# snap-stanford/KGWAS

Measured on AMD Instinct MI355X. Metric: edges aggregated/sec (full fast-mode KG minibatch training; epoch time in config), higher is better.
Workload: dtype f32

## Files before the change

kgwas_amd/csrc/kgw_dense_linear.h:

```cpp
#pragma once

namespace {

constexpr int LBM = 128, LBN = 128, LBK = 32, LPAD = 33;

struct LinArgs {
    const float* X; int64_t ldx;
    const float* W; int64_t ldw;
    const float* bias;
    const float* mask;
    int64_t ldm;
    float* Y; int64_t ldy;
    int64_t rows; int K, N;
    int relu, w_kn;
    const int32_t* rows_dev;
};

__device__ __forceinline__ int64_t lin_rows_eff(const LinArgs& a) {
    if (!a.rows_dev) return a.rows;
    const int64_t r = *a.rows_dev;
    return r < 0 ? 0 : (r < a.rows ? r : a.rows);
}

__device__ __forceinline__ void lin_zero_padding(const LinArgs& a, int64_t rows_eff, int64_t tid, int64_t nthreads) {
// ... 919 lines not shown
            const int idx = tid + 256 * it;
            const int k = idx & 127, n4 = (idx >> 7) * 4;
            Wl[(n4 + 0) * WST + k] = wv[it].x; Wl[(n4 + 1) * WST + k] = wv[it].y;
            Wl[(n4 + 2) * WST + k] = wv[it].z; Wl[(n4 + 3) * WST + k] = wv[it].w;
        }
    }
    __syncthreads();
    f32x4 bw[2][16];
#pragma unroll
    for (int t = 0; t < 2; ++t)
#pragma unroll
        for (int q = 0; q < 16; ++q) bw[t][q] = *(const f32x4*)(Wl + (t * 32 + li) * WST + lk * 64 + 4 * q);
    const float* w2 = Wl + (64 + li) * WST + lk * 64;
    const float* w3 = Wl + (96 + li) * WST + lk * 64;
    f32x16 accw[4];
#pragma unroll
    for (int t = 0; t < 4; ++t)
#pragma unroll
        for (int e = 0; e < 16; ++e) accw[t][e] = 0.f;
    const int K1 = a.K1;
    int tile = (int)blockIdx.x * 4 + wave;
    f32x4 xa[16];
    int src_cur;
    {
        int64_t r = (int64_t)(tile < ntiles ? tile : ntiles - 1) * 32 + li;
        if (r >= rows) r = rows - 1;
        src_cur = a.in_ids ? a.in_ids[r] : 0;
        const float* xp = a.dH2 + (a.in_ids ? (int64_t)(src_cur < 0 ? 0 : src_cur) : r) * a.ldd + lk * 64;
#pragma unroll
        for (int q = 0; q < 16; ++q) xa[q] = *(const f32x4*)(xp + 4 * q);
    }
    for (; tile < ntiles; tile += nw) {
        const int64_t r0 = (int64_t)tile * 32;
        const int64_t row = r0 + li;
        const bool live = row < rows && src_cur >= 0;
        const int64_t rc = row < rows ? row : rows - 1;
        const float* xn;
        {
            int nt = tile + nw;
            if (nt >= ntiles) nt = ntiles - 1;
            int64_t r = (int64_t)nt * 32 + li;
            if (r >= rows) r = rows - 1;
            src_cur = a.in_ids ? a.in_ids[r] : 0;
            xn = a.dH2 + (a.in_ids ? (int64_t)(src_cur < 0 ? 0 : src_cur) : r) * a.ldd + lk * 64;
        }
        float xs[16];
#pragma unroll
        for (int s2 = 0; s2 < 16; ++s2) {
            const int64_t rr = r0 + 2 * s2 + lk;
            float v = 0.f;
            if (rr < rows) v = li < K1 ? a.X[rr * a.ldx + li] : (li == K1 ? 1.f : 0.f);
            xs[s2] = v;
        }
        const float* mp = a.H1 + rc * a.ldm + 4 * lk;
        unsigned mb[2] = {0u, 0u};
        f32x4 mv[4];
#define KGW_MLPB_MFETCH(T)                                                                                \
        _Pragma("unroll") for (int g = 0; g < 4; ++g) mv[g] = *(const f32x4*)(mp + (T) * 32 + 8 * g);
#define KGW_MLPB_MBITS(T)                                                                                 \
        _Pragma("unroll") for (int g = 0; g < 4; ++g) {                                                  \
            const int b0 = ((T) & 1) * 16 + 4 * g;                                                        \
            mb[(T) >> 1] |= (mv[g].x > 0.f ? 1u : 0u) << (b0 + 0);                                        \
            mb[(T) >> 1] |= (mv[g].y > 0.f ? 1u : 0u) << (b0 + 1);                                        \
            mb[(T) >> 1] |= (mv[g].z > 0.f ? 1u : 0u) << (b0 + 2);                                        \
            mb[(T) >> 1] |= (mv[g].w > 0.f ? 1u : 0u) << (b0 + 3);                                        \
        }
        f32x16 acc[4];
#pragma unroll
        for (int t = 0; t < 4; ++t)
#pragma unroll
            for (int e = 0; e < 16; ++e) acc[t][e] = 0.f;
        f32x4 b2n = *(const f32x4*)w2, b3n = *(const f32x4*)w3;
#pragma unroll
        for (int q = 0; q < 16; ++q) {
            if (q == 0) { KGW_MLPB_MFETCH(0) }
            if (q == 3) { KGW_MLPB_MBITS(0) KGW_MLPB_MFETCH(1) }
            if (q == 6) { KGW_MLPB_MBITS(1) KGW_MLPB_MFETCH(2) }
            if (q == 10) { KGW_MLPB_MBITS(2) KGW_MLPB_MFETCH(3) }
            if (q == 14) { KGW_MLPB_MBITS(3) }
            const f32x4 b2 = b2n, b3 = b3n;
            if (q + 1 < 16) { b2n = *(const f32x4*)(w2 + 4 * (q + 1)); b3n = *(const f32x4*)(w3 + 4 * (q + 1)); }
#define KGW_MLPB_STEP(C)                                                                                  \
            acc[0] = __builtin_amdgcn_mfma_f32_32x32x2f32(bw[0][q].C, xa[q].C, acc[0], 0, 0, 0);          \
            acc[1] = __builtin_amdgcn_mfma_f32_32x32x2f32(bw[1][q].C, xa[q].C, acc[1], 0, 0, 0);          \
            acc[2] = __builtin_amdgcn_mfma_f32_32x32x2f32(b2.C, xa[q].C, acc[2], 0, 0, 0);                \
            acc[3] = __builtin_amdgcn_mfma_f32_32x32x2f32(b3.C, xa[q].C, acc[3], 0, 0, 0);
            KGW_MLPB_STEP(x) KGW_MLPB_STEP(y) KGW_MLPB_STEP(z) KGW_MLPB_STEP(w)
#undef KGW_MLPB_STEP
            if (q == 7) {
                __builtin_amdgcn_sched_barrier(0);
#pragma unroll
                for (int qq = 0; qq < 8; ++qq) xa[qq] = *(const f32x4*)(xn + 4 * qq);
                __builtin_amdgcn_sched_barrier(0);
            }
        }
#undef KGW_MLPB_MFETCH
#undef KGW_MLPB_MBITS
        if (!live) { mb[0] = 0u; mb[1] = 0u; }
        __builtin_amdgcn_sched_barrier(0);
#pragma unroll
        for (int qq = 8; qq < 16; ++qq) xa[qq] = *(const f32x4*)(xn + 4 * qq);
        __builtin_amdgcn_sched_barrier(0);
#pragma unroll
        for (int t = 0; t < 4; ++t)
#pragma unroll
            for (int g = 0; g < 4; ++g) {
                const unsigned m4 = mb[t >> 1] >> (((t & 1) << 4) + 4 * g);
                f32x4 v;
                v.x = (m4 & 1u) ? acc[t][4 * g + 0] : 0.f; v.y = (m4 & 2u) ? acc[t][4 * g + 1] : 0.f;
                v.z = (m4 & 4u) ? acc[t][4 * g + 2] : 0.f; v.w = (m4 & 8u) ? acc[t][4 * g + 3] : 0.f;
                *(f32x4*)(Tw + li * TST + t * 32 + 8 * g + 4 * lk) = v;
                if (a.dZ && row < rows) *(f32x4*)(a.dZ + row * a.ldz + t * 32 + 8 * g + 4 * lk) = v;
            }
        __asm__ volatile("s_waitcnt lgkmcnt(0)" ::: "memory");
#pragma unroll
        for (int s2 = 0; s2 < 16; ++s2) {
            const float* tp = Tw + (2 * s2 + lk) * TST + li;
#pragma unroll
            for (int t = 0; t < 4; ++t)
                accw[t] = __builtin_amdgcn_mfma_f32_32x32x2f32(xs[s2], tp[t * 32], accw[t], 0, 0, 0);
        }
        __asm__ volatile("s_waitcnt lgkmcnt(0)" ::: "memory");
    }
    __syncthreads();
    float* R = Tl;
#pragma unroll
    for (int t = 0; t < 4; ++t)
#pragma unroll
        for (int e = 0; e < 16; ++e) R[wave * 4096 + (t * 16 + e) * 64 + lane] = accw[t][e];
    __syncthreads();
    for (int f = tid; f < 4096; f += 256)
        a.part[(int64_t)blockIdx.x * 4096 + f] = (R[f] + R[4096 + f]) + (R[2 * 4096 + f] + R[3 * 4096 + f]);
}

constexpr int TS2 = 68;

template <bool PACK>
__global__ void __launch_bounds__(256) __attribute__((amdgpu_waves_per_eu(1, 1))) k_mlp2_bwd_first3(Mlp2BwdArgs a) {
    extern __shared__ __attribute__((aligned(16))) float lds[];
    uint4* W2p = (uint4*)lds;
    float* Tl = lds + M3_W2_U4 * 4;
    const int tid = threadIdx.x, lane = tid & 63, wave = tid >> 6;
    const int li = lane & 31, lk = lane >> 5;
    const unsigned sgn = (li & 1) ? 0x80000000u : 0u;
    int64_t rows = a.rows;
    if (a.rows_dev) { const int64_t r = *a.rows_dev; rows = r < 0 ? 0 : (r < a.rows ? r : a.rows); }
    if (rows == 0) {
        for (int f = tid; f < 4096; f += 256) a.part[(int64_t)blockIdx.x * 4096 + f] = 0.f;
        return;
    }
    const int ntiles = (int)((rows + 31) / 32);
    const int nw = (int)gridDim.x * 4;
    float* Tw = Tl + wave * 32 * TS2;
    for (int idx = tid; idx < 8 * 4 * 64; idx += 256) {
        const int ln = idx & 63, jt = (idx >> 6) & 3, s_ = idx >> 8;
        const float* wp = a.W2 + (int64_t)(64 * (ln >> 5) + 8 * s_) * a.ldw + 32 * jt + (ln & 31);
        float x[8];
#pragma unroll
        for (int i = 0; i < 8; ++i) x[i] = wp[(int64_t)i * a.ldw];
        uint4 p1, p2, p3;
        kgw_split3x8(x, p1, p2, p3);
        uint4* o = W2p + ((s_ * 3) * 4 + jt) * 64 + ln;
        o[0] = p1; o[4 * 64] = p2; o[8 * 64] = p3;
    }
    __syncthreads();
    const uint4* w2p = W2p + lane;
    f32x16 accw[4];
#pragma unroll
    for (int t = 0; t < 4; ++t)
#pragma unroll
        for (int e = 0; e < 16; ++e) accw[t][e] = 0.f;
    const int K1 = a.K1;
    int tile = (int)blockIdx.x * 4 + wave;
    f32x4 xa[16];
    int src_cur;
    {
        int64_t r = (int64_t)(tile < ntiles ? tile : ntiles - 1) * 32 + li;
        if (r >= rows) r = rows - 1;
        src_cur = a.in_ids ? a.in_ids[r] : 0;
        const float* xp = a.dH2 + (a.in_ids ? (int64_t)(src_cur < 0 ? 0 : src_cur) : r) * a.ldd + lk * 64;
#pragma unroll
        for (int q = 0; q < 16; ++q) xa[q] = *(const f32x4*)(xp + 4 * q);
    }
#define KGW_MLPB_BITS(MV, MB)                                                                            \
    _Pragma("unroll") for (int t_ = 0; t_ < 4; ++t_) _Pragma("unroll") for (int g = 0; g < 4; ++g) {    \
        const int b0 = (t_ & 1) * 16 + 4 * g;                                                            \
        MB[t_ >> 1] |= (MV[t_][g].x > 0.f ? 1u : 0u) << (b0 + 0);                                        \
        MB[t_ >> 1] |= (MV[t_][g].y > 0.f ? 1u : 0u) << (b0 + 1);                                        \
        MB[t_ >> 1] |= (MV[t_][g].z > 0.f ? 1u : 0u) << (b0 + 2);                                        \
        MB[t_ >> 1] |= (MV[t_][g].w > 0.f ? 1u : 0u) << (b0 + 3);                                        \
    }
    unsigned mb[2] = {0u, 0u};
    {
        int64_t r = (int64_t)(tile < ntiles ? tile : ntiles - 1) * 32 + li;
        if (r >= rows) r = rows - 1;
        const float* mp = a.H1 + r * a.ldm + 4 * lk;
        f32x4 mv[4][4];
#pragma unroll
        for (int t_ = 0; t_ < 4; ++t_)
#pragma unroll
            for (int g = 0; g < 4; ++g) mv[t_][g] = *(const f32x4*)(mp + t_ * 32 + 8 * g);
        KGW_MLPB_BITS(mv, mb)
    }
    for (; tile < ntiles; tile += nw) {
        const int64_t r0 = (int64_t)tile * 32;
        const int64_t row = r0 + li;
        const bool live = row < rows && src_cur >= 0;
        const int64_t rc = row < rows ? row : rows - 1;
        const float* xn;
        {
            int nt = tile + nw;
            if (nt >= ntiles) nt = ntiles - 1;
            int64_t r = (int64_t)nt * 32 + li;
            if (r >= rows) r = rows - 1;
            src_cur = a.in_ids ? a.in_ids[r] : 0;
            xn = a.dH2 + (a.in_ids ? (int64_t)(src_cur < 0 ? 0 : src_cur) : r) * a.ldd + lk * 64;
        }
        float xs[16];
#pragma unroll
        for (int s2 = 0; s2 < 16; ++s2) {
            const int64_t rr = r0 + 2 * s2 + lk;
            float v = 0.f;
            if (rr < rows) v = li < K1 ? a.X[rr * a.ldx + li] : (li == K1 ? 1.f : 0.f);
            xs[s2] = v;
        }
        f32x4 mvn[4][4];
        {
            int nt = tile + nw;
            if (nt >= ntiles) nt = ntiles - 1;
            int64_t r = (int64_t)nt * 32 + li;
            if (r >= rows) r = rows - 1;
            const float* mpn = a.H1 + r * a.ldm + 4 * lk;
#pragma unroll
            for (int t_ = 0; t_ < 4; ++t_)
#pragma unroll
                for (int g = 0; g < 4; ++g) mvn[t_][g] = *(const f32x4*)(mpn + t_ * 32 + 8 * g);
        }
        f32x16 acc[4];
#pragma unroll
        for (int t = 0; t < 4; ++t)
#pragma unroll
            for (int e = 0; e < 16; ++e) acc[t][e] = 0.f;
#pragma unroll
        for (int s_ = 0; s_ < 8; ++s_) {
            const f32x4 u = xa[2 * s_], v = xa[2 * s_ + 1];
            const float h[8] = {kgw_fxor(u.x, sgn), kgw_fxor(u.y, sgn), kgw_fxor(u.z, sgn), kgw_fxor(u.w, sgn),
                                kgw_fxor(v.x, sgn), kgw_fxor(v.y, sgn), kgw_fxor(v.z, sgn), kgw_fxor(v.w, sgn)};
            uint4 p1, p2, p3;
            kgw_split3x8(h, p1, p2, p3);
            const kgw_bf8 hb[3] = {__builtin_bit_cast(kgw_bf8, p1), __builtin_bit_cast(kgw_bf8, p2), __builtin_bit_cast(kgw_bf8, p3)};
            kgw_bf8 wa[3][4];
#pragma unroll
            for (int p = 0; p < 3; ++p)
#pragma unroll
                for (int jt = 0; jt < 4; ++jt) wa[p][jt] = __builtin_bit_cast(kgw_bf8, w2p[((s_ * 3 + p) * 4 + jt) * 64]);
            constexpr int TW[6] = {0, 2, 1, 0, 1, 0}, TH[6] = {2, 0, 1, 1, 0, 0};
#pragma unroll
            for (int t6 = 0; t6 < 6; ++t6)
#pragma unroll
                for (int jt = 0; jt < 4; ++jt)
                    acc[jt] = __builtin_amdgcn_mfma_f32_32x32x16_bf16(wa[TW[t6]][jt], hb[TH[t6]], acc[jt], 0, 0, 0);
            if (s_ == 3) {
                __builtin_amdgcn_sched_barrier(0);
#pragma unroll
                for (int qq = 0; qq < 8; ++qq) xa[qq] = *(const f32x4*)(xn + 4 * qq);
                __builtin_amdgcn_sched_barrier(0);
            }
        }
        if (!live) { mb[0] = 0u; mb[1] = 0u; }
        __builtin_amdgcn_sched_barrier(0);
#pragma unroll
        for (int qq = 8; qq < 16; ++qq) xa[qq] = *(const f32x4*)(xn + 4 * qq);
        __builtin_amdgcn_sched_barrier(0);
#pragma unroll
        for (int hh = 0; hh < 2; ++hh) {
#pragma unroll
            for (int t = 2 * hh; t < 2 * hh + 2; ++t)
#pragma unroll
                for (int g = 0; g < 4; ++g) {
                    const unsigned m4 = mb[t >> 1] >> (((t & 1) << 4) + 4 * g);
                    f32x4 v;
                    v.x = (m4 & 1u) ? kgw_fxor(acc[t][4 * g + 0], sgn) : 0.f; v.y = (m4 & 2u) ? kgw_fxor(acc[t][4 * g + 1], sgn) : 0.f;
                    v.z = (m4 & 4u) ? kgw_fxor(acc[t][4 * g + 2], sgn) : 0.f; v.w = (m4 & 8u) ? kgw_fxor(acc[t][4 * g + 3], sgn) : 0.f;
                    *(f32x4*)(Tw + li * TS2 + (t - 2 * hh) * 32 + 8 * g + 4 * lk) = v;
                    if (a.dZ && row < rows) *(f32x4*)(a.dZ + row * a.ldz + t * 32 + 8 * g + 4 * lk) = v;
                }
            __asm__ volatile("s_waitcnt lgkmcnt(0)" ::: "memory");
            if (PACK) {
                const bool neg = a.flip && ((tile / a.flip) & 1);
#pragma unroll
                for (int it = 0; it < 4; ++it) {
                    const int ntl = it & 1, j = it >> 1;
                    const float* tp = Tw + (16 * j + 8 * lk) * TS2 + 32 * ntl + li;
                    float x[8];
#pragma unroll
                    for (int i = 0; i < 8; ++i) x[i] = neg ? -tp[i * TS2] : tp[i * TS2];
                    uint4 p1, p2, p3;
                    kgw_split3x8(x, p1, p2, p3);
                    uint4* o = a.packed + (((int64_t)tile * 2 + j) * 3 * 4 + (2 * hh + ntl)) * 64 + lane;
                    o[0] = p1; o[4 * 64] = p2; o[8 * 64] = p3;
                }
            }
#pragma unroll
            for (int s2 = 0; s2 < 16; ++s2) {
                const float* tp = Tw + (2 * s2 + lk) * TS2 + li;
#pragma unroll
                for (int t = 0; t < 2; ++t)
                    accw[2 * hh + t] = __builtin_amdgcn_mfma_f32_32x32x2f32(xs[s2], tp[t * 32], accw[2 * hh + t], 0, 0, 0);
            }
            __asm__ volatile("s_waitcnt lgkmcnt(0)" ::: "memory");
        }
        mb[0] = 0u; mb[1] = 0u;
        KGW_MLPB_BITS(mvn, mb)
    }
#undef KGW_MLPB_BITS
    __syncthreads();
    float* R = lds;
#pragma unroll
    for (int t = 0; t < 4; ++t)
#pragma unroll
        for (int e = 0; e < 16; ++e) R[wave * 4096 + (t * 16 + e) * 64 + lane] = accw[t][e];
    __syncthreads();
    for (int f = tid; f < 4096; f += 256)
        a.part[(int64_t)blockIdx.x * 4096 + f] = (R[f] + R[4096 + f]) + (R[2 * 4096 + f] + R[3 * 4096 + f]);
}

__global__ void __launch_bounds__(1024) k_mlp2_bwd_fold(const float* __restrict__ part, int nblk, int K1, float* __restrict__ dW1,
                                                        int64_t ldw, float* __restrict__ db1) {
    __shared__ float sm[1024];
    const int fl = threadIdx.x & 63, g = threadIdx.x >> 6;
    const int f = blockIdx.x * 64 + fl;
    float s4[4] = {0.f, 0.f, 0.f, 0.f};
    int q = 0;
    for (int b = g; b < nblk; b += 16, ++q) s4[q & 3] += part[(int64_t)b * 4096 + f];
    sm[threadIdx.x] = (s4[0] + s4[1]) + (s4[2] + s4[3]);
    __syncthreads();
    if (g == 0) {
        float sv = 0.f;
#pragma unroll
        for (int k = 0; k < 16; k += 4) sv += (sm[k * 64 + fl] + sm[(k + 1) * 64 + fl]) + (sm[(k + 2) * 64 + fl] + sm[(k + 3) * 64 + fl]);
        const int lane = f & 63, e = (f >> 6) & 15, t = f >> 10;
        const int k = (e & 3) + 8 * (e >> 2) + 4 * (lane >> 5), col = 32 * t + (lane & 31);
        if (k < K1) dW1[(int64_t)col * ldw + k] = sv;
        else if (k == K1) db1[col] = sv;
    }
}

template <bool WKN, bool MASK>
__global__ void __launch_bounds__(256) __attribute__((amdgpu_waves_per_eu(2, 2))) k_linear_wreg_half(LinArgs a_) {
    extern __shared__ __attribute__((aligned(16))) float lds[];
    LinArgs a = a_;
    {
        const int64_t re = lin_rows_eff(a_);
        lin_zero_padding(a_, re, (int64_t)blockIdx.x * 256 + threadIdx.x, (int64_t)gridDim.x * 256);
        a.rows = re;
        if ((int64_t)blockIdx.x * 2 * 32 >= re) return;
// ... 315 lines not shown
```

kgwas_amd/csrc/kgw_dense_optim.h:

```cpp
#pragma once

namespace {
__global__ void __launch_bounds__(256) k_scatter_relu_rows(const float* __restrict__ g, const int32_t* __restrict__ g2l,
                                                           const float* __restrict__ h, int64_t n_rows,
                                                           float* __restrict__ dz, float* __restrict__ part) {
    __shared__ float4 red[8][32];
    const int r8 = threadIdx.x >> 5, c4 = threadIdx.x & 31;
    float4 acc = make_float4(0.f, 0.f, 0.f, 0.f);
    for (int64_t r = (int64_t)blockIdx.x * 8 + r8; r < n_rows; r += (int64_t)gridDim.x * 8) {
        const int pos = g2l[r];
        float4 v = make_float4(0.f, 0.f, 0.f, 0.f);
        if (pos >= 0) {
            const float4 gv = ((const float4*)g)[(int64_t)pos * 32 + c4];
            const float4 hv = ((const float4*)h)[r * 32 + c4];
            v.x = hv.x > 0.f ? gv.x : 0.f; v.y = hv.y > 0.f ? gv.y : 0.f;
            v.z = hv.z > 0.f ? gv.z : 0.f; v.w = hv.w > 0.f ? gv.w : 0.f;
        }
        ((float4*)dz)[r * 32 + c4] = v;
        acc.x += v.x; acc.y += v.y; acc.z += v.z; acc.w += v.w;
    }
    red[r8][c4] = acc;
    __syncthreads();
    if (r8 == 0) {
#pragma unroll
// ... 10 lines not shown
    for (; b + 56 < nblk; b += 64) {
#pragma unroll
        for (int k = 0; k < 8; ++k) s[k] += part[(int64_t)(b + 8 * k) * 128 + c];
    }
    for (int k = 0; b < nblk; b += 8, ++k) s[k & 7] += part[(int64_t)b * 128 + c];
    sm[gq][c] = ((s[0] + s[1]) + (s[2] + s[3])) + ((s[4] + s[5]) + (s[6] + s[7]));
    __syncthreads();
    if (gq == 0) {
        float t = 0.f;
#pragma unroll
        for (int k = 0; k < 8; ++k) t += sm[k][c];
        out[c] = t;
    }
}
}

extern "C" int64_t kgw_scatter_relu_rows_workspace_floats(int64_t n_rows) {
    int64_t nblk = (n_rows + 7) / 8;
    if (nblk > 256) nblk = 256;
    return (nblk > 0 ? nblk : 1) * 128;
}

extern "C" int kgw_scatter_relu_rows(const float* g, const int32_t* g2l, const float* h, int64_t n_rows, float* dz,
                                     float* colsum, float* workspace, kgw_stream_t stream_) {
    if (!g2l || !h || !dz || !colsum || !workspace) return KGW_E_NULL;
    if (n_rows <= 0) return KGW_E_RANGE;
    if (!aligned16(h) || !aligned16(dz) || !aligned16(workspace) || (g && !aligned16(g))) return KGW_E_UNSUPPORTED;
    int64_t nblk = (n_rows + 7) / 8;
    if (nblk > 256) nblk = 256;
    k_scatter_relu_rows<<<(int)nblk, 256, 0, (hipStream_t)stream_>>>(g, g2l, h, n_rows, dz, workspace);
    KGW_LAUNCH_CHECK();
    k_colsum_fold<<<1, 1024, 0, (hipStream_t)stream_>>>(workspace, (int)nblk, colsum);
    KGW_LAUNCH_CHECK();
    return KGW_OK;
}

namespace {

constexpr int ADAM_MAX = 64;
struct AdamTab {
    float* p[ADAM_MAX]; const float* g[ADAM_MAX]; float* m[ADAM_MAX]; float* v[ADAM_MAX];
    int64_t off[ADAM_MAX + 1];
    int64_t coff[ADAM_MAX + 1];
    unsigned char vec[ADAM_MAX];
    int n;
};

__device__ __forceinline__ void adam_update(float& p, float g0, float& m, float& v, float wd, float b1, float b2, float eps,
                                            float step_size, float bc2_sqrt) {
#pragma clang fp contract(off)
    const float g = fmaf(wd, p, g0);
    m = m + (1.0f - b1) * (g - m);
    v = v * b2 + (1.0f - b2) * g * g;
    const float denom = sqrtf(v) / bc2_sqrt + eps;
    p = p - step_size * (m / denom);
}

__global__ void __launch_bounds__(256) k_adam(AdamTab T, int32_t* step, float lr, float b1, float b2, float eps, float wd) {
    const int t_now = *step + 1;
    const float bc1 = 1.0f - powf(b1, (float)t_now);
    const float bc2 = 1.0f - powf(b2, (float)t_now);
    const float step_size = lr / bc1;
    const float bc2_sqrt = sqrtf(bc2);
    const int64_t units = T.coff[T.n];
    for (int64_t c = blockIdx.x; c < units; c += gridDim.x) {
        int lo = 0, hi = T.n;
        while (hi - lo > 1) { const int mid = (lo + hi) >> 1; if (T.coff[mid] <= c) lo = mid; else hi = mid; }
        const int64_t n = T.off[lo + 1] - T.off[lo];
        const int64_t j = (c - T.coff[lo]) * 1024 + (int64_t)threadIdx.x * 4;
        float* __restrict__ P = T.p[lo];
        const float* __restrict__ G = T.g[lo];
        float* __restrict__ M = T.m[lo];
        float* __restrict__ V = T.v[lo];
        if (j + 4 <= n && T.vec[lo]) {
            float4 p = *(float4*)(P + j), m = *(float4*)(M + j), v = *(float4*)(V + j);
            const float4 g0 = *(const float4*)(G + j);
            float pe[4] = {p.x, p.y, p.z, p.w}, ge[4] = {g0.x, g0.y, g0.z, g0.w}, me[4] = {m.x, m.y, m.z, m.w}, ve[4] = {v.x, v.y, v.z, v.w};
#pragma unroll
            for (int e = 0; e < 4; ++e) adam_update(pe[e], ge[e], me[e], ve[e], wd, b1, b2, eps, step_size, bc2_sqrt);
            *(float4*)(M + j) = make_float4(me[0], me[1], me[2], me[3]);
            *(float4*)(V + j) = make_float4(ve[0], ve[1], ve[2], ve[3]);
            *(float4*)(P + j) = make_float4(pe[0], pe[1], pe[2], pe[3]);
        } else {
            for (int64_t i = j; i < n && i < j + 4; ++i) {
                float p = P[i], m = M[i], v = V[i];
                adam_update(p, G[i], m, v, wd, b1, b2, eps, step_size, bc2_sqrt);
                M[i] = m; V[i] = v; P[i] = p;
            }
        }
    }
}

__global__ void k_adam_tick(int32_t* step) { if (threadIdx.x == 0 && blockIdx.x == 0) *step += 1; }

}

static int adam_launch(int32_t n_tensors, float* const* params, const float* const* grads, float* const* exp_avg,
                       float* const* exp_avg_sq, const int64_t* numel, int32_t* step_dev, float lr, float beta1,
                       float beta2, float eps, float weight_decay, bool tick, kgw_stream_t stream_) {
    if (n_tensors == 0) return KGW_OK;
    if (!params || !grads || !exp_avg || !exp_avg_sq || !numel || !step_dev) return KGW_E_NULL;
    if (n_tensors < 0 || n_tensors > ADAM_MAX) return KGW_E_RANGE;
    AdamTab T;
    T.n = n_tensors;
    T.off[0] = 0;
    T.coff[0] = 0;
    for (int i = 0; i < n_tensors; ++i) {
        if (!params[i] || !grads[i] || !exp_avg[i] || !exp_avg_sq[i] || numel[i] < 0) return KGW_E_NULL;
        T.p[i] = params[i]; T.g[i] = grads[i]; T.m[i] = exp_avg[i]; T.v[i] = exp_avg_sq[i];
        T.off[i + 1] = T.off[i] + numel[i];
        T.coff[i + 1] = T.coff[i] + (numel[i] + 1023) / 1024;
        T.vec[i] = (((uintptr_t)params[i] | (uintptr_t)grads[i] | (uintptr_t)exp_avg[i] | (uintptr_t)exp_avg_sq[i]) & 15) == 0;
    }
    hipStream_t st = (hipStream_t)stream_;
    int64_t g = T.coff[n_tensors];
    if (g > 4 * KGW_GRID) g = 4 * KGW_GRID;
    if (g < 1) g = 1;
    k_adam<<<(int)g, 256, 0, st>>>(T, step_dev, lr, beta1, beta2, eps, weight_decay);
    KGW_LAUNCH_CHECK();
    if (tick) {
        k_adam_tick<<<1, 64, 0, st>>>(step_dev);
        KGW_LAUNCH_CHECK();
    }
    return KGW_OK;
}

extern "C" int kgw_adam(int32_t n_tensors, float* const* params, const float* const* grads, float* const* exp_avg,
                        float* const* exp_avg_sq, const int64_t* numel, int32_t* step_dev, float lr, float beta1,
                        float beta2, float eps, float weight_decay, kgw_stream_t stream_) {
    return adam_launch(n_tensors, params, grads, exp_avg, exp_avg_sq, numel, step_dev, lr, beta1, beta2, eps, weight_decay, true,
                       stream_);
}

extern "C" int kgw_adam_notick(int32_t n_tensors, float* const* params, const float* const* grads, float* const* exp_avg,
                               float* const* exp_avg_sq, const int64_t* numel, int32_t* step_dev, float lr, float beta1,
                               float beta2, float eps, float weight_decay, kgw_stream_t stream_) {
    return adam_launch(n_tensors, params, grads, exp_avg, exp_avg_sq, numel, step_dev, lr, beta1, beta2, eps, weight_decay, false,
                       stream_);
}

namespace {

struct AdamFTab {
    float* p[KGW_ADAM_FUSED_MAX]; float* g[KGW_ADAM_FUSED_MAX]; float* m[KGW_ADAM_FUSED_MAX]; float* v[KGW_ADAM_FUSED_MAX];
    int64_t off[KGW_ADAM_FUSED_MAX + 1];
    int64_t coff[KGW_ADAM_FUSED_MAX + 1];
    unsigned char vec[KGW_ADAM_FUSED_MAX];
    unsigned char src_of[KGW_ADAM_FUSED_MAX];
    KgwGradSrc src[KGW_ADAM_FUSED_SRC];
    int n;
};
struct AdamTail { const KgwBatchMeta* meta; int64_t* stats; int32_t* done; int n_layers, n_hops; };

__device__ __forceinline__ float adam_src_sum(const KgwGradSrc& S, int64_t i, bool valid, int fl, int G, float* sm) {
    const int nblk = S.nblk;
    if (S.kind == KGW_GRAD_TN) {
        const int MT = S.MT, NT = S.NT;
        const int64_t FRAG = (int64_t)MT * NT * 1024;
        int m, n;
        if (!S.c_transposed) { m = (int)(i / S.N); n = (int)(i - (int64_t)m * S.N); }
        else                 { n = (int)(i / S.M); m = (int)(i - (int64_t)n * S.M); }
        const int by = m / (32 * MT), rm = m - by * 32 * MT, ta = rm % MT, ti = rm / MT;
        const int bz = n / (32 * NT), rn = n - bz * 32 * NT, tb = rn % NT, tj = rn / NT;
        const int lane = tj + 32 * ((ti >> 2) & 1), e = (ti & 3) + 4 * (ti >> 3);
        const float* p = S.ws + ((int64_t)bz * S.gy + by) * nblk * FRAG + ((ta * NT + tb) * 16 + e) * 64 + lane;
        float s8[8] = {0.f, 0.f, 0.f, 0.f, 0.f, 0.f, 0.f, 0.f};
        if (valid) {
            int b = G;
            for (; b + 28 < nblk; b += 32) {
#pragma unroll
                for (int q = 0; q < 8; ++q) s8[q] += p[(int64_t)(b + 4 * q) * FRAG];
            }
            for (int q = 0; b < nblk; b += 4, ++q) s8[q & 7] += p[(int64_t)b * FRAG];
        }
        sm[G * 64 + fl] = ((s8[0] + s8[1]) + (s8[2] + s8[3])) + ((s8[4] + s8[5]) + (s8[6] + s8[7]));
        __syncthreads();
        return (sm[fl] + sm[64 + fl]) + (sm[128 + fl] + sm[192 + fl]);
    }
    if (S.kind == KGW_GRAD_TN_COLSUM) {
        const int NC = 32 * S.MT, NG = 256 / NC;
        const int m = (int)i, by = m / NC, c = m - by * NC;
        const float* p = S.ws + (int64_t)by * nblk * NC + c;
        for (int gq = G; gq < NG; gq += 4) {
            float s4[4] = {0.f, 0.f, 0.f, 0.f};
            if (valid) {
                int b = gq;
                for (; b + 3 * NG < nblk; b += 4 * NG) {
#pragma unroll
                    for (int q = 0; q < 4; ++q) s4[q] += p[(int64_t)(b + q * NG) * NC];
                }
                for (int q = 0; b < nblk; b += NG, ++q) s4[q & 3] += p[(int64_t)b * NC];
            }
            sm[gq * 64 + fl] = (s4[0] + s4[1]) + (s4[2] + s4[3]);
        }
        __syncthreads();
        float t = 0.f;
        for (int q = 0; q < NG; ++q) t += sm[q * 64 + fl];
        return t;
    }
    {
        int col, k;
        if (S.kind == KGW_GRAD_MLP2_W) { col = (int)(i / S.K1); k = (int)(i - (int64_t)col * S.K1); }
        else                           { col = (int)i; k = S.K1; }
        const int t = col >> 5, lane = (col & 31) + 32 * ((k >> 2) & 1), e = (k & 3) + 4 * (k >> 3);
        const float* p = S.ws + (t * 16 + e) * 64 + lane;
#pragma unroll
        for (int u = 0; u < 4; ++u) {
            const int gg = G + 4 * u;
            float s4[4] = {0.f, 0.f, 0.f, 0.f};
            if (valid) {
                int b = gg;
                for (; b + 48 < nblk; b += 64) {
                    float x[4];
#pragma unroll
                    for (int j = 0; j < 4; ++j) x[j] = p[(int64_t)(b + 16 * j) * 4096];
#pragma unroll
                    for (int j = 0; j < 4; ++j) s4[j] += x[j];
                }
#pragma unroll
                for (int j = 0; j < 4; ++j)
                    if (b + 16 * j < nblk) s4[j] += p[(int64_t)(b + 16 * j) * 4096];
            }
            sm[gg * 64 + fl] = (s4[0] + s4[1]) + (s4[2] + s4[3]);
        }
        __syncthreads();
        float sv = 0.f;
#pragma unroll
        for (int k4 = 0; k4 < 16; k4 += 4) sv += (sm[k4 * 64 + fl] + sm[(k4 + 1) * 64 + fl]) + (sm[(k4 + 2) * 64 + fl] + sm[(k4 + 3) * 64 + fl]);
        return sv;
    }
}

template <bool UPD>
__global__ void __launch_bounds__(256) k_adam_fused(AdamFTab T, AdamTail Z, int32_t* step, float lr, float b1, float b2, float eps,
                                                    float wd) {
    __shared__ float sm[32 * 33];
    const int t_now = UPD ? *step + 1 : 1;
    const float bc1 = 1.0f - powf(b1, (float)t_now);
    const float bc2 = 1.0f - powf(b2, (float)t_now);
    const float step_size = lr / bc1;
    const float bc2_sqrt = sqrtf(bc2);
    const int64_t units = T.coff[T.n];
    const int fl = threadIdx.x & 63, G = threadIdx.x >> 6;
    for (int64_t c = blockIdx.x; c < units; c += gridDim.x) {
        int lo = 0, hi = T.n;
        while (hi - lo > 1) { const int mid = (lo + hi) >> 1; if (T.coff[mid] <= c) lo = mid; else hi = mid; }
        const int64_t n = T.off[lo + 1] - T.off[lo];
        float* __restrict__ P = T.p[lo];
        float* __restrict__ Gr = T.g[lo];
        float* __restrict__ M = T.m[lo];
        float* __restrict__ V = T.v[lo];
        const int si = T.src_of[lo];
        if (si != 255 && T.src[si].kind == KGW_GRAD_G3T) {
            const KgwGradSrc& S = T.src[si];
            const int64_t u = c - T.coff[lo];
            const int64_t Mr = S.M, r0 = (u >> 2) * 32;
            const int cb = (int)(u & 3) * 32;
            float (*tl)[33] = (float (*)[33])sm;
            {
                const int r = threadIdx.x >> 3, c4 = threadIdx.x & 7;
                const float4* w = (const float4*)S.ws + (r0 + r) * 32 + (cb >> 2) + c4;
                const int64_t ks = Mr * 32;
                float4 a4 = w[0];
                int k = 1;
                for (; k + 3 < S.nblk; k += 4) {
                    float4 x[4];
#pragma unroll
                    for (int q = 0; q < 4; ++q) x[q] = w[(int64_t)(k + q) * ks];
#pragma unroll
                    for (int q = 0; q < 4; ++q) { a4.x += x[q].x; a4.y += x[q].y; a4.z += x[q].z; a4.w += x[q].w; }
                }
                for (; k < S.nblk; ++k) {
                    const float4 x = w[(int64_t)k * ks];
                    a4.x += x.x; a4.y += x.y; a4.z += x.z; a4.w += x.w;
                }
                tl[r][4 * c4] = a4.x; tl[r][4 * c4 + 1] = a4.y; tl[r][4 * c4 + 2] = a4.z; tl[r][4 * c4 + 3] = a4.w;
            }
            __syncthreads();
            {
                const int r = threadIdx.x & 31;
                float pq[4], mq[4], vq[4], gq[4];
                if constexpr (!UPD) {
#pragma unroll
                    for (int q = 0; q < 4; ++q) {
                        const int col = (threadIdx.x >> 5) + 8 * q;
                        const int64_t i = (int64_t)(cb + col) * Mr + r0 + r;
                        const float g = tl[r][col];
                        Gr[i] = g; P[i] = g;
                    }
                    __syncthreads();
                    continue;
                }
#pragma unroll
                for (int q = 0; q < 4; ++q) {
                    const int col = (threadIdx.x >> 5) + 8 * q;
                    const int64_t i = (int64_t)(cb + col) * Mr + r0 + r;
                    gq[q] = tl[r][col];
                    pq[q] = P[i]; mq[q] = M[i]; vq[q] = V[i];
                }
#pragma unroll
                for (int q = 0; q < 4; ++q) {
                    const int col = (threadIdx.x >> 5) + 8 * q;
                    const int64_t i = (int64_t)(cb + col) * Mr + r0 + r;
                    adam_update(pq[q], gq[q], mq[q], vq[q], wd, b1, b2, eps, step_size, bc2_sqrt);
                    Gr[i] = gq[q]; M[i] = mq[q]; V[i] = vq[q]; P[i] = pq[q];
                    tl[r][col] = pq[q];
                }
            }
            __syncthreads();
            if (S.packed && threadIdx.x < 128) {
                const int j = threadIdx.x >> 6, lane = threadIdx.x & 63;
                const int64_t ch = r0 >> 5;
                float x[8];
#pragma unroll
                for (int e = 0; e < 8; ++e) x[e] = tl[16 * j + 8 * (lane >> 5) + e][lane & 31];
                if (S.flip && ((ch / S.flip) & 1)) {
#pragma unroll
                    for (int e = 0; e < 8; ++e) x[e] = -x[e];
                }
                uint4 p1, p2, p3;
                kgw_split3x8(x, p1, p2, p3);
                uint4* o = (uint4*)S.packed + ((ch * 2 + j) * 3 * 4 + (cb >> 5)) * 64 + lane;
                o[0] = p1; o[4 * 64] = p2; o[8 * 64] = p3;
            }
            __syncthreads();
            continue;
        }
        if (si != 255) {
            const int64_t i = (c - T.coff[lo]) * 64 + fl;
            const bool valid = i < n;
            const float gs = adam_src_sum(T.src[si], i, valid, fl, G, sm);
            if (G == 0 && valid) {
                Gr[i] = gs;
                if constexpr (UPD) {
                    float p = P[i], m = M[i], v = V[i];
                    adam_update(p, gs, m, v, wd, b1, b2, eps, step_size, bc2_sqrt);
                    M[i] = m; V[i] = v; P[i] = p;
                } else {
                    P[i] = gs;
                }
            }
            __syncthreads();
            continue;
        }
        const int64_t j = (c - T.coff[lo]) * 1024 + (int64_t)threadIdx.x * 4;
        if constexpr (!UPD) {
            if (j + 4 <= n && T.vec[lo]) *(float4*)(P + j) = *(const float4*)(Gr + j);
            else for (int64_t i = j; i < n && i < j + 4; ++i) P[i] = Gr[i];
            continue;
        }
        if (j + 4 <= n && T.vec[lo]) {
            float4 p = *(float4*)(P + j), m = *(float4*)(M + j), v = *(float4*)(V + j);
            const float4 g0 = *(const float4*)(Gr + j);
            float pe[4] = {p.x, p.y, p.z, p.w}, ge[4] = {g0.x, g0.y, g0.z, g0.w}, me[4] = {m.x, m.y, m.z, m.w}, ve[4] = {v.x, v.y, v.z, v.w};
#pragma unroll
            for (int e = 0; e < 4; ++e) adam_update(pe[e], ge[e], me[e], ve[e], wd, b1, b2, eps, step_size, bc2_sqrt);
            *(float4*)(M + j) = make_float4(me[0], me[1], me[2], me[3]);
            *(float4*)(V + j) = make_float4(ve[0], ve[1], ve[2], ve[3]);
            *(float4*)(P + j) = make_float4(pe[0], pe[1], pe[2], pe[3]);
        } else {
            for (int64_t i = j; i < n && i < j + 4; ++i) {
                float p = P[i], m = M[i], v = V[i];
                adam_update(p, Gr[i], m, v, wd, b1, b2, eps, step_size, bc2_sqrt);
                M[i] = m; V[i] = v; P[i] = p;
            }
        }
    }
    if constexpr (!UPD) return;
    __syncthreads();
    if (threadIdx.x == 0) {
        const int slot = (int)(blockIdx.x & 63), in_slot = ((int)gridDim.x - slot + 63) >> 6;
        const int n_slots = (int)gridDim.x < 64 ? (int)gridDim.x : 64;
        int32_t* c1 = Z.done + 32 * (1 + slot);
        if (__hip_atomic_fetch_add(c1, 1, __ATOMIC_RELAXED, __HIP_MEMORY_SCOPE_AGENT) == in_slot - 1) {
            __hip_atomic_store(c1, 0, __ATOMIC_RELAXED, __HIP_MEMORY_SCOPE_AGENT);
            if (__hip_atomic_fetch_add(Z.done, 1, __ATOMIC_RELAXED, __HIP_MEMORY_SCOPE_AGENT) == n_slots - 1) {
                __hip_atomic_store(Z.done, 0, __ATOMIC_RELAXED, __HIP_MEMORY_SCOPE_AGENT);
                *step = t_now;
                if (Z.meta) {
                    const KgwBatchMeta* Mt = Z.meta;
                    for (int t = 0; t < Z.n_layers; ++t) Z.stats[t] += Mt->n_edges[t];
                    Z.stats[Z.n_layers] += Mt->edge_end[Z.n_hops - 1];
                    Z.stats[Z.n_layers + 1] |= Mt->error;
                }
            }
        }
    }
}

}

static int adam_fused_table(AdamFTab& T, int32_t n_tensors, float* const* params, float* const* grads, float* const* exp_avg,
                            float* const* exp_avg_sq, const int64_t* numel, const KgwGradSrc* src);

extern "C" int kgw_adam_fused(int32_t n_tensors, float* const* params, float* const* grads, float* const* exp_avg,
                              float* const* exp_avg_sq, const int64_t* numel, const KgwGradSrc* src, int32_t* step_dev, float lr,
                              float beta1, float beta2, float eps, float weight_decay, const KgwBatchMeta* meta_dev,
                              int32_t n_layers, int32_t n_hops, int64_t* stats, int32_t* done_counter, kgw_stream_t stream_) {
    if (n_tensors < 0 || n_tensors > KGW_ADAM_FUSED_MAX) return KGW_E_RANGE;
    if (!step_dev || !done_counter) return KGW_E_NULL;
    if (n_tensors > 0 && (!params || !grads || !exp_avg || !exp_avg_sq || !numel)) return KGW_E_NULL;
    if (meta_dev && (!stats || n_layers < 1 || n_layers > KGW_MAX_LAYERS || n_hops < 1 || n_hops > n_layers)) return KGW_E_RANGE;
    AdamFTab T;
    const int rc = adam_fused_table(T, n_tensors, params, grads, exp_avg, exp_avg_sq, numel, src);
    if (rc != KGW_OK) return rc;
    AdamTail Z{meta_dev, stats, done_counter, n_layers, n_hops};
    int64_t g = T.coff[n_tensors];
    if (g > 4 * KGW_GRID) g = 4 * KGW_GRID;
    if (g < 1) g = 1;
    k_adam_fused<true><<<(int)g, 256, 0, (hipStream_t)stream_>>>(T, Z, step_dev, lr, beta1, beta2, eps, weight_decay);
    KGW_LAUNCH_CHECK();
    return KGW_OK;
}

extern "C" int kgw_grad_finish(int32_t n_tensors, float* const* dst, float* const* grads, const int64_t* numel, const KgwGradSrc* src,
                               kgw_stream_t stream_) {
    if (n_tensors < 0 || n_tensors > KGW_ADAM_FUSED_MAX) return KGW_E_RANGE;
    if (n_tensors == 0) return KGW_OK;
    if (!dst || !grads || !numel) return KGW_E_NULL;
    AdamFTab T;
    const int rc = adam_fused_table(T, n_tensors, dst, grads, dst, dst, numel, src);
    if (rc != KGW_OK) return rc;
    for (int i = 0; i < n_tensors; ++i)
        if (src && src[i].kind == KGW_GRAD_G3T && src[i].packed) return KGW_E_UNSUPPORTED;
    AdamTail Z{};
    int64_t g = T.coff[n_tensors];
    if (g > 4 * KGW_GRID) g = 4 * KGW_GRID;
    k_adam_fused<false><<<(int)g, 256, 0, (hipStream_t)stream_>>>(T, Z, nullptr, 0.f, 0.f, 0.f, 0.f, 0.f);
    KGW_LAUNCH_CHECK();
    return KGW_OK;
}

static int adam_fused_table(AdamFTab& T, int32_t n_tensors, float* const* params, float* const* grads, float* const* exp_avg,
                            float* const* exp_avg_sq, const int64_t* numel, const KgwGradSrc* src) {
    T.n = n_tensors;
    T.off[0] = 0;
    T.coff[0] = 0;
    int nsrc = 0;
    for (int i = 0; i < n_tensors; ++i) {
        if (!params[i] || !grads[i] || !exp_avg[i] || !exp_avg_sq[i] || numel[i] < 0) return KGW_E_NULL;
        T.p[i] = params[i]; T.g[i] = grads[i]; T.m[i] = exp_avg[i]; T.v[i] = exp_avg_sq[i];
        T.src_of[i] = 255;
        int64_t per = 1024;
        if (src && src[i].kind != KGW_GRAD_DIRECT) {
            const KgwGradSrc& S = src[i];
            if (nsrc >= KGW_ADAM_FUSED_SRC) return KGW_E_RANGE;
            if (!S.ws || S.nblk < 1) return KGW_E_NULL;
            if (S.kind == KGW_GRAD_TN) {
                if (S.MT < 1 || S.NT < 1 || S.MT * S.NT > 16 || (256 % (32 * S.MT)) || (int64_t)S.M * S.N != numel[i]) return KGW_E_RANGE;
            } else if (S.kind == KGW_GRAD_TN_COLSUM) {
                if (S.MT < 1 || (256 % (32 * S.MT)) || S.M != numel[i]) return KGW_E_RANGE;
            } else if (S.kind == KGW_GRAD_MLP2_W) {
                if (S.K1 < 1 || S.K1 > 31 || (int64_t)128 * S.K1 != numel[i]) return KGW_E_RANGE;
            } else if (S.kind == KGW_GRAD_MLP2_B) {
                if (S.K1 < 0 || S.K1 > 31 || numel[i] != 128) return KGW_E_RANGE;
            } else if (S.kind == KGW_GRAD_G3T) {
                if (S.M < 32 || (S.M & 31) || (int64_t)128 * S.M != numel[i] || S.flip < 0 || (S.flip & (S.flip - 1))) return KGW_E_RANGE;
                if (((uintptr_t)S.ws | (uintptr_t)S.packed) & 15) return KGW_E_UNSUPPORTED;
            } else {
                return KGW_E_RANGE;
            }
            T.src[nsrc] = S;
            T.src_of[i] = (unsigned char)nsrc++;
            per = S.kind == KGW_GRAD_G3T ? 1024 : 64;
        }
        T.off[i + 1] = T.off[i] + numel[i];
        T.coff[i + 1] = T.coff[i] + (numel[i] + per - 1) / per;
        T.vec[i] = (((uintptr_t)params[i] | (uintptr_t)grads[i] | (uintptr_t)exp_avg[i] | (uintptr_t)exp_avg_sq[i]) & 15) == 0;
    }
    return KGW_OK;
}
```

Baseline: 1.088 billion.

## Hoist global loads ahead of dependent work in MLP backward and Adam reductions

In the MLP2 backward kernel, the W2 weight loads, the first-tile H1 mask loads and the dH2 loads are all issued together up front, before the packing and the LDS sync, so their latencies overlap. In the Adam partial-sum reduction, the strided slab loops are replaced by a templated helper that issues a whole group of loads before any accumulation. It uses a scheduling barrier and opaque offsets to stop the compiler from interleaving or merging them. The P/M/V optimizer state loads are also moved ahead of the reduction so they overlap it, and G is made wave-uniform with readfirstlane. The cost is higher register pressure, which may lower occupancy or cause spills.

Result: no change. 1.097 billion (median of 6 runs) (+0.8%).

```diff
diff --git a/kgwas_amd/csrc/kgw_dense_linear.h b/kgwas_amd/csrc/kgw_dense_linear.h
--- a/kgwas_amd/csrc/kgw_dense_linear.h
+++ b/kgwas_amd/csrc/kgw_dense_linear.h
@@ -1095,14 +1095,38 @@
     const int ntiles = (int)((rows + 31) / 32);
     const int nw = (int)gridDim.x * 4;
     float* Tw = Tl + wave * 32 * TS2;
-    for (int idx = tid; idx < 8 * 4 * 64; idx += 256) {
+    int tile = (int)blockIdx.x * 4 + wave;
+    f32x4 xa[16];
+    int src_cur;
+    f32x4 mv0[4][4];
+    float wx[8][8];
+    {
+        int64_t r = (int64_t)(tile < ntiles ? tile : ntiles - 1) * 32 + li;
+        if (r >= rows) r = rows - 1;
+        src_cur = a.in_ids ? a.in_ids[r] : 0;
+        const float* mp = a.H1 + r * a.ldm + 4 * lk;
+#pragma unroll
+        for (int t_ = 0; t_ < 4; ++t_)
+#pragma unroll
+            for (int g = 0; g < 4; ++g) mv0[t_][g] = *(const f32x4*)(mp + t_ * 32 + 8 * g);
+#pragma unroll
+        for (int it = 0; it < 8; ++it) {
+            const int idx = tid + 256 * it;
+            const int ln = idx & 63, jt = (idx >> 6) & 3, s_ = idx >> 8;
+            const float* wp = a.W2 + (int64_t)(64 * (ln >> 5) + 8 * s_) * a.ldw + 32 * jt + (ln & 31);
+#pragma unroll
+            for (int i = 0; i < 8; ++i) wx[it][i] = wp[(int64_t)i * a.ldw];
+        }
+        const float* xp = a.dH2 + (a.in_ids ? (int64_t)(src_cur < 0 ? 0 : src_cur) : r) * a.ldd + lk * 64;
+#pragma unroll
+        for (int q = 0; q < 16; ++q) xa[q] = *(const f32x4*)(xp + 4 * q);
+    }
+#pragma unroll
+    for (int it = 0; it < 8; ++it) {
+        const int idx = tid + 256 * it;
         const int ln = idx & 63, jt = (idx >> 6) & 3, s_ = idx >> 8;
-        const float* wp = a.W2 + (int64_t)(64 * (ln >> 5) + 8 * s_) * a.ldw + 32 * jt + (ln & 31);
-        float x[8];
-#pragma unroll
-        for (int i = 0; i < 8; ++i) x[i] = wp[(int64_t)i * a.ldw];
         uint4 p1, p2, p3;
-        kgw_split3x8(x, p1, p2, p3);
+        kgw_split3x8(wx[it], p1, p2, p3);
         uint4* o = W2p + ((s_ * 3) * 4 + jt) * 64 + ln;
         o[0] = p1; o[4 * 64] = p2; o[8 * 64] = p3;
     }
@@ -1114,17 +1138,6 @@
 #pragma unroll
         for (int e = 0; e < 16; ++e) accw[t][e] = 0.f;
     const int K1 = a.K1;
-    int tile = (int)blockIdx.x * 4 + wave;
-    f32x4 xa[16];
-    int src_cur;
-    {
-        int64_t r = (int64_t)(tile < ntiles ? tile : ntiles - 1) * 32 + li;
-        if (r >= rows) r = rows - 1;
-        src_cur = a.in_ids ? a.in_ids[r] : 0;
-        const float* xp = a.dH2 + (a.in_ids ? (int64_t)(src_cur < 0 ? 0 : src_cur) : r) * a.ldd + lk * 64;
-#pragma unroll
-        for (int q = 0; q < 16; ++q) xa[q] = *(const f32x4*)(xp + 4 * q);
-    }
 #define KGW_MLPB_BITS(MV, MB)                                                                            \
     _Pragma("unroll") for (int t_ = 0; t_ < 4; ++t_) _Pragma("unroll") for (int g = 0; g < 4; ++g) {    \
         const int b0 = (t_ & 1) * 16 + 4 * g;                                                            \
@@ -1134,17 +1147,7 @@
         MB[t_ >> 1] |= (MV[t_][g].w > 0.f ? 1u : 0u) << (b0 + 3);                                        \
     }
     unsigned mb[2] = {0u, 0u};
-    {
-        int64_t r = (int64_t)(tile < ntiles ? tile : ntiles - 1) * 32 + li;
-        if (r >= rows) r = rows - 1;
-        const float* mp = a.H1 + r * a.ldm + 4 * lk;
-        f32x4 mv[4][4];
-#pragma unroll
-        for (int t_ = 0; t_ < 4; ++t_)
-#pragma unroll
-            for (int g = 0; g < 4; ++g) mv[t_][g] = *(const f32x4*)(mp + t_ * 32 + 8 * g);
-        KGW_MLPB_BITS(mv, mb)
-    }
+    KGW_MLPB_BITS(mv0, mb)
     for (; tile < ntiles; tile += nw) {
         const int64_t r0 = (int64_t)tile * 32;
         const int64_t row = r0 + li;
diff --git a/kgwas_amd/csrc/kgw_dense_optim.h b/kgwas_amd/csrc/kgw_dense_optim.h
--- a/kgwas_amd/csrc/kgw_dense_optim.h
+++ b/kgwas_amd/csrc/kgw_dense_optim.h
@@ -186,6 +186,39 @@
 };
 struct AdamTail { const KgwBatchMeta* meta; int64_t* stats; int32_t* done; int n_layers, n_hops; };
 
+#define KGW_OPAQUE_OFF(O) __asm__ volatile("" : "+s"(O));
+
+__device__ __forceinline__ void kgw_acc(float& a, const float& x) { a += x; }
+__device__ __forceinline__ void kgw_acc(float4& a, const float4& x) { a.x += x.x; a.y += x.y; a.z += x.z; a.w += x.w; }
+
+template <int NACC, int NL, bool FULL, typename T>
+__device__ __forceinline__ void adam_slab_group(const T* __restrict__ p, int64_t& off, int64_t d, int n, T (&s)[NACC]) {
+    static_assert(NL % NACC == 0 && (NACC & (NACC - 1)) == 0, "a group is whole rounds of the accumulators");
+    T x[NL];
+#pragma unroll
+    for (int q = 0; q < NL; ++q) {
+        x[q] = p[off];
+        off += FULL || q + 1 < n ? d : 0;
+        KGW_OPAQUE_OFF(off)
+    }
+    __builtin_amdgcn_sched_barrier(0);
+#pragma unroll
+    for (int q = 0; q < NL; ++q)
+        if (FULL || q < n) kgw_acc(s[q & (NACC - 1)], x[q]);
+}
+
+template <int NACC, int N, int NS, typename T>
+__device__ __forceinline__ void adam_slab_sums(const T* __restrict__ p, int64_t stride, int start, int step, int nblk, T (&s)[NACC]) {
+    const int cnt = start < nblk ? (nblk - start + step - 1) / step : 0;
+    int64_t off = (int64_t)start * stride;
+    const int64_t d = (int64_t)step * stride;
+    int m = 0;
+    for (; m + N <= cnt; m += N) adam_slab_group<NACC, N, true>(p, off, d, N, s);
+    const int rem = cnt - m;
+    if (rem > NS) adam_slab_group<NACC, N, false>(p, off, d, rem, s);
+    else if (rem > 0) adam_slab_group<NACC, NS, false>(p, off, d, rem, s);
+}
+
 __device__ __forceinline__ float adam_src_sum(const KgwGradSrc& S, int64_t i, bool valid, int fl, int G, float* sm) {
     const int nblk = S.nblk;
     if (S.kind == KGW_GRAD_TN) {
@@ -199,14 +232,7 @@
         const int lane = tj + 32 * ((ti >> 2) & 1), e = (ti & 3) + 4 * (ti >> 3);
         const float* p = S.ws + ((int64_t)bz * S.gy + by) * nblk * FRAG + ((ta * NT + tb) * 16 + e) * 64 + lane;
         float s8[8] = {0.f, 0.f, 0.f, 0.f, 0.f, 0.f, 0.f, 0.f};
-        if (valid) {
-            int b = G;
-            for (; b + 28 < nblk; b += 32) {
-#pragma unroll
-                for (int q = 0; q < 8; ++q) s8[q] += p[(int64_t)(b + 4 * q) * FRAG];
-            }
-            for (int q = 0; b < nblk; b += 4, ++q) s8[q & 7] += p[(int64_t)b * FRAG];
-        }
+        if (valid) adam_slab_sums<8, 32, 8>(p, FRAG, G, 4, nblk, s8);
         sm[G * 64 + fl] = ((s8[0] + s8[1]) + (s8[2] + s8[3])) + ((s8[4] + s8[5]) + (s8[6] + s8[7]));
         __syncthreads();
         return (sm[fl] + sm[64 + fl]) + (sm[128 + fl] + sm[192 + fl]);
@@ -217,14 +243,7 @@
         const float* p = S.ws + (int64_t)by * nblk * NC + c;
         for (int gq = G; gq < NG; gq += 4) {
             float s4[4] = {0.f, 0.f, 0.f, 0.f};
-            if (valid) {
-                int b = gq;
-                for (; b + 3 * NG < nblk; b += 4 * NG) {
-#pragma unroll
-                    for (int q = 0; q < 4; ++q) s4[q] += p[(int64_t)(b + q * NG) * NC];
-                }
-                for (int q = 0; b < nblk; b += NG, ++q) s4[q & 3] += p[(int64_t)b * NC];
-            }
+            if (valid) adam_slab_sums<4, 32, 8>(p, NC, gq, NG, nblk, s4);
             sm[gq * 64 + fl] = (s4[0] + s4[1]) + (s4[2] + s4[3]);
         }
         __syncthreads();
@@ -238,25 +257,10 @@
         else                           { col = (int)i; k = S.K1; }
         const int t = col >> 5, lane = (col & 31) + 32 * ((k >> 2) & 1), e = (k & 3) + 4 * (k >> 3);
         const float* p = S.ws + (t * 16 + e) * 64 + lane;
-#pragma unroll
-        for (int u = 0; u < 4; ++u) {
-            const int gg = G + 4 * u;
-            float s4[4] = {0.f, 0.f, 0.f, 0.f};
-            if (valid) {
-                int b = gg;
-                for (; b + 48 < nblk; b += 64) {
-                    float x[4];
-#pragma unroll
-                    for (int j = 0; j < 4; ++j) x[j] = p[(int64_t)(b + 16 * j) * 4096];
-#pragma unroll
-                    for (int j = 0; j < 4; ++j) s4[j] += x[j];
-                }
-#pragma unroll
-                for (int j = 0; j < 4; ++j)
-                    if (b + 16 * j < nblk) s4[j] += p[(int64_t)(b + 16 * j) * 4096];
-            }
-            sm[gg * 64 + fl] = (s4[0] + s4[1]) + (s4[2] + s4[3]);
-        }
+        float s16[16] = {0.f, 0.f, 0.f, 0.f, 0.f, 0.f, 0.f, 0.f, 0.f, 0.f, 0.f, 0.f, 0.f, 0.f, 0.f, 0.f};
+        if (valid) adam_slab_sums<16, 64, 16>(p, 4096, G, 4, nblk, s16);
+#pragma unroll
+        for (int u = 0; u < 4; ++u) sm[(G + 4 * u) * 64 + fl] = (s16[u] + s16[u + 4]) + (s16[u + 8] + s16[u + 12]);
         __syncthreads();
         float sv = 0.f;
 #pragma unroll
@@ -275,7 +279,7 @@
     const float step_size = lr / bc1;
     const float bc2_sqrt = sqrtf(bc2);
     const int64_t units = T.coff[T.n];
-    const int fl = threadIdx.x & 63, G = threadIdx.x >> 6;
+    const int fl = threadIdx.x & 63, G = __builtin_amdgcn_readfirstlane((int)(threadIdx.x >> 6));
     for (int64_t c = blockIdx.x; c < units; c += gridDim.x) {
         int lo = 0, hi = T.n;
         while (hi - lo > 1) { const int mid = (lo + hi) >> 1; if (T.coff[mid] <= c) lo = mid; else hi = mid; }
@@ -291,29 +295,27 @@
             const int64_t Mr = S.M, r0 = (u >> 2) * 32;
             const int cb = (int)(u & 3) * 32;
             float (*tl)[33] = (float (*)[33])sm;
+            float pq[4] = {0.f, 0.f, 0.f, 0.f}, mq[4] = {0.f, 0.f, 0.f, 0.f}, vq[4] = {0.f, 0.f, 0.f, 0.f}, gq[4];
+            if constexpr (UPD) {
+                const int r = threadIdx.x & 31;
+#pragma unroll
+                for (int q = 0; q < 4; ++q) {
+                    const int col = (threadIdx.x >> 5) + 8 * q;
+                    const int64_t i = (int64_t)(cb + col) * Mr + r0 + r;
+                    pq[q] = P[i]; mq[q] = M[i]; vq[q] = V[i];
+                }
+            }
             {
                 const int r = threadIdx.x >> 3, c4 = threadIdx.x & 7;
                 const float4* w = (const float4*)S.ws + (r0 + r) * 32 + (cb >> 2) + c4;
                 const int64_t ks = Mr * 32;
-                float4 a4 = w[0];
-                int k = 1;
-                for (; k + 3 < S.nblk; k += 4) {
-                    float4 x[4];
-#pragma unroll
-                    for (int q = 0; q < 4; ++q) x[q] = w[(int64_t)(k + q) * ks];
-#pragma unroll
-                    for (int q = 0; q < 4; ++q) { a4.x += x[q].x; a4.y += x[q].y; a4.z += x[q].z; a4.w += x[q].w; }
-                }
-                for (; k < S.nblk; ++k) {
-                    const float4 x = w[(int64_t)k * ks];
-                    a4.x += x.x; a4.y += x.y; a4.z += x.z; a4.w += x.w;
-                }
-                tl[r][4 * c4] = a4.x; tl[r][4 * c4 + 1] = a4.y; tl[r][4 * c4 + 2] = a4.z; tl[r][4 * c4 + 3] = a4.w;
+                float4 a4[1] = {w[0]};
+                adam_slab_sums<1, 16, 4>(w, ks, 1, 1, S.nblk, a4);
+                tl[r][4 * c4] = a4[0].x; tl[r][4 * c4 + 1] = a4[0].y; tl[r][4 * c4 + 2] = a4[0].z; tl[r][4 * c4 + 3] = a4[0].w;
             }
             __syncthreads();
             {
                 const int r = threadIdx.x & 31;
-                float pq[4], mq[4], vq[4], gq[4];
                 if constexpr (!UPD) {
 #pragma unroll
                     for (int q = 0; q < 4; ++q) {
@@ -326,12 +328,7 @@
                     continue;
                 }
 #pragma unroll
-                for (int q = 0; q < 4; ++q) {
-                    const int col = (threadIdx.x >> 5) + 8 * q;
-                    const int64_t i = (int64_t)(cb + col) * Mr + r0 + r;
-                    gq[q] = tl[r][col];
-                    pq[q] = P[i]; mq[q] = M[i]; vq[q] = V[i];
-                }
+                for (int q = 0; q < 4; ++q) gq[q] = tl[r][(threadIdx.x >> 5) + 8 * q];
 #pragma unroll
                 for (int q = 0; q < 4; ++q) {
                     const int col = (threadIdx.x >> 5) + 8 * q;
@@ -363,11 +360,14 @@
         if (si != 255) {
             const int64_t i = (c - T.coff[lo]) * 64 + fl;
             const bool valid = i < n;
+            float p = 0.f, m = 0.f, v = 0.f;
+            if constexpr (UPD) {
+                if (G == 0 && valid) { p = P[i]; m = M[i]; v = V[i]; }
+            }
             const float gs = adam_src_sum(T.src[si], i, valid, fl, G, sm);
             if (G == 0 && valid) {
                 Gr[i] = gs;
                 if constexpr (UPD) {
-                    float p = P[i], m = M[i], v = V[i];
                     adam_update(p, gs, m, v, wd, b1, b2, eps, step_size, bc2_sqrt);
                     M[i] = m; V[i] = v; P[i] = p;
                 } else {
```
